# prismformore/Multi-Task-Transformer

Hardware: NVIDIA H100
Metric: images/sec (higher is better)
Workload: dtype bf16x3 (split-bf16 operands, fp32 accumulate)

## Files before the change

multi-task-transformer_b200/csrc/attention5_tc.cu:

```cuda
#include <math.h>

#include "host_common.h"
#include "ptx.cuh"

namespace mtt {

constexpr int kA5ConsumerWGs = 3;
constexpr int kA5Rows = 64 * kA5ConsumerWGs;
constexpr int kA5Threads = 128 + 128 * kA5ConsumerWGs;
constexpr uint32_t kA5QTile = kA5Rows * 64 * 2;
constexpr uint32_t kA5KVTile = 64 * 64 * 2;
constexpr int kA5Stages = 3;

struct Attn5Params {
  int B, N, H, T;
  float scale_log2;
  __nv_bfloat16* out_hi;
  __nv_bfloat16* out_lo;
  float* prompt_logits;
};

template <int NSPLIT>
__global__ void __launch_bounds__(kA5Threads, 1)
attention5_kernel(const __grid_constant__ CUtensorMap tmq_hi, const __grid_constant__ CUtensorMap tmq_lo,
                  const __grid_constant__ CUtensorMap tmk_hi, const __grid_constant__ CUtensorMap tmk_lo,
                  const Attn5Params p) {
  extern __shared__ uint8_t smem_raw[];
  uint8_t* smem = reinterpret_cast<uint8_t*>((reinterpret_cast<uintptr_t>(smem_raw) + 1023) &
                                             ~static_cast<uintptr_t>(1023));
  uint8_t* sQ = smem;
  uint8_t* sK = sQ + NSPLIT * kA5QTile;
  uint8_t* sV = sK + kA5Stages * NSPLIT * kA5KVTile;
  uint64_t* bars = reinterpret_cast<uint64_t*>(sV + kA5Stages * NSPLIT * kA5KVTile);
  uint64_t* q_full = bars;
  uint64_t* k_full = bars + 1;
  uint64_t* k_empty = k_full + kA5Stages;
  uint64_t* v_full = k_empty + kA5Stages;
  uint64_t* v_empty = v_full + kA5Stages;

  const int tid = threadIdx.x;
  const int warp = tid >> 5;
  const int lane = tid & 31;
  const int C = p.H * 64;
  const int nkv = (p.N + 63) / 64;
  const int qt = blockIdx.x / (p.B * p.H);
  const int h = blockIdx.x % p.H;
  const int b = (blockIdx.x / p.H) % p.B;
  const int n_act = min(kA5ConsumerWGs, (p.N - qt * kA5Rows + 63) / 64);

  if (tid == 0) {
    tma_prefetch_desc(&tmq_hi);
    tma_prefetch_desc(&tmk_hi);
    if (NSPLIT == 2) {
      tma_prefetch_desc(&tmq_lo);
      tma_prefetch_desc(&tmk_lo);
    }
    mbar_init(q_full, 1);
    for (int s = 0; s < kA5Stages; ++s) {
      mbar_init(&k_full[s], 1);
      mbar_init(&k_empty[s], 4 * n_act);
      mbar_init(&v_full[s], 1);
      mbar_init(&v_empty[s], 4 * n_act);
    }
    fence_barrier_init();
  }
  __syncthreads();

  if (warp < 4) {
    setmaxnreg_dec<24>();
    if (warp != 0) return;
    if (elect_one()) {
      mbar_arrive_expect_tx(q_full, NSPLIT * kA5QTile);
      tma_load_3d(sQ, &tmq_hi, q_full, h * 64, qt * kA5Rows, b);
      if (NSPLIT == 2) tma_load_3d(sQ + kA5QTile, &tmq_lo, q_full, h * 64, qt * kA5Rows, b);
    }
    __syncwarp();
    for (int j = 0; j < nkv; ++j) {
      const int s = j % kA5Stages;
      const uint32_t ph = (j / kA5Stages) & 1;
      mbar_wait(&k_empty[s], ph ^ 1);
      if (elect_one()) {
        uint8_t* dk = sK + s * NSPLIT * kA5KVTile;
        mbar_arrive_expect_tx(&k_full[s], NSPLIT * kA5KVTile);
        tma_load_3d(dk, &tmk_hi, &k_full[s], C + h * 64, j * 64, b);
        if (NSPLIT == 2) tma_load_3d(dk + kA5KVTile, &tmk_lo, &k_full[s], C + h * 64, j * 64, b);
      }
      __syncwarp();
      mbar_wait(&v_empty[s], ph ^ 1);
      if (elect_one()) {
        uint8_t* dv = sV + s * NSPLIT * kA5KVTile;
        mbar_arrive_expect_tx(&v_full[s], NSPLIT * kA5KVTile);
        tma_load_3d(dv, &tmk_hi, &v_full[s], 2 * C + h * 64, j * 64, b);
        if (NSPLIT == 2) tma_load_3d(dv + kA5KVTile, &tmk_lo, &v_full[s], 2 * C + h * 64, j * 64, b);
      }
      __syncwarp();
    }
    return;
  }

  setmaxnreg_inc<160>();
  const int cw = (warp >> 2) - 1;
  if (cw >= n_act) return;
  const int rloc = cw * 64 + (warp & 3) * 16 + (lane >> 2);
  const int col0 = 2 * (lane & 3);
  const uint32_t q_hi = smem_u32(sQ) + (uint32_t)cw * 64 * 128;
  const uint32_t q_lo = q_hi + kA5QTile;
  const float sl2 = p.scale_log2;

  float o[32];
#pragma unroll
  for (int i = 0; i < 32; ++i) o[i] = 0.f;
  float m_run[2] = {-INFINITY, -INFINITY};
  float l_run[2] = {0.f, 0.f};

  mbar_wait(q_full, 0);
  for (int j = 0; j < nkv; ++j) {
    const int s = j % kA5Stages;
    const uint32_t ph = (j / kA5Stages) & 1;
    const int kn = min(64, p.N - j * 64);

    float sc[32];
#pragma unroll
    for (int i = 0; i < 32; ++i) sc[i] = 0.f;
    mbar_wait(&k_full[s], ph);
    const uint32_t k_hi = smem_u32(sK + s * NSPLIT * kA5KVTile), k_lo = k_hi + kA5KVTile;
    wgmma_fence_regs(sc);
    wgmma_fence();
#pragma unroll
    for (int ks = 0; ks < 4; ++ks) {
      const uint64_t qdh = gmma_desc_sw128(q_hi + ks * 32), kdh = gmma_desc_sw128(k_hi + ks * 32);
      wgmma_ss_n64<0>(sc, qdh, kdh, 1);
      if (NSPLIT == 2) {
        wgmma_ss_n64<0>(sc, qdh, gmma_desc_sw128(k_lo + ks * 32), 1);
        wgmma_ss_n64<0>(sc, gmma_desc_sw128(q_lo + ks * 32), kdh, 1);
      }
    }
    wgmma_commit();
    wgmma_wait<0>();
    wgmma_fence_regs(sc);
    __syncwarp();
    if (lane == 0) mbar_arrive(&k_empty[s]);

    if (p.prompt_logits) {
#pragma unroll
      for (int hh = 0; hh < 2; ++hh) {
        const int q_row = qt * kA5Rows + rloc + 8 * hh;
        if (q_row < p.T) {
          float* ex = p.prompt_logits + (((long long)b * p.H + h) * p.T + q_row) * p.N + j * 64;
#pragma unroll
          for (int i = 0; i < 8; ++i) {
            const int c = 8 * i + col0;
            if (c < kn) ex[c] = sc[4 * i + 2 * hh];
            if (c + 1 < kn) ex[c + 1] = sc[4 * i + 2 * hh + 1];
          }
        }
      }
    }

    float alpha[2];
#pragma unroll
    for (int hh = 0; hh < 2; ++hh) {
      float mx = -INFINITY;
#pragma unroll
      for (int i = 0; i < 8; ++i) {
#pragma unroll
        for (int e = 0; e < 2; ++e) {
          if (8 * i + col0 + e >= kn) sc[4 * i + 2 * hh + e] = -INFINITY;
          mx = fmaxf(mx, sc[4 * i + 2 * hh + e]);
        }
      }
      mx = fmaxf(mx, __shfl_xor_sync(0xffffffffu, mx, 1));
      mx = fmaxf(mx, __shfl_xor_sync(0xffffffffu, mx, 2));
      const float m_new = fmaxf(m_run[hh], mx * sl2);
      alpha[hh] = ex2_approx(m_run[hh] - m_new);
      m_run[hh] = m_new;
      float sum = 0.f;
#pragma unroll
      for (int i = 0; i < 8; ++i) {
#pragma unroll
        for (int e = 0; e < 2; ++e) {
          const float pv = ex2_approx(fmaf(sc[4 * i + 2 * hh + e], sl2, -m_new));
          sc[4 * i + 2 * hh + e] = pv;
          sum += pv;
        }
      }
      l_run[hh] = l_run[hh] * alpha[hh] + sum;
    }

    uint32_t ph_[4][4], pl_[4][4];
#pragma unroll
    for (int kk = 0; kk < 4; ++kk) {
#pragma unroll
      for (int r = 0; r < 4; ++r) {
        const int i = 2 * kk + (r >> 1), hh = r & 1;
        if (NSPLIT == 2) split_pack2(sc[4 * i + 2 * hh], sc[4 * i + 2 * hh + 1], ph_[kk][r], pl_[kk][r]);
        else ph_[kk][r] = pack_bf16x2(sc[4 * i + 2 * hh], sc[4 * i + 2 * hh + 1]);
      }
    }
    mbar_wait(&v_full[s], ph);
    const uint32_t v_hi = smem_u32(sV + s * NSPLIT * kA5KVTile), v_lo = v_hi + kA5KVTile;
    float pvb[32];
#pragma unroll
    for (int i = 0; i < 32; ++i) pvb[i] = 0.f;
    wgmma_fence_regs(pvb);
    wgmma_fence();
#pragma unroll
    for (int kk = 0; kk < 4; ++kk) {
      const uint64_t vdh = gmma_desc_sw128(v_hi + kk * 2048);
      wgmma_rs_n64<1>(pvb, ph_[kk], vdh, kk > 0 ? 1 : 0);
      if (NSPLIT == 2) {
        wgmma_rs_n64<1>(pvb, ph_[kk], gmma_desc_sw128(v_lo + kk * 2048), 1);
        wgmma_rs_n64<1>(pvb, pl_[kk], vdh, 1);
      }
    }
    wgmma_commit();
    wgmma_wait<0>();
    wgmma_fence_regs(pvb);
#pragma unroll
    for (int i = 0; i < 8; ++i)
#pragma unroll
      for (int r = 0; r < 4; ++r) o[4 * i + r] = fmaf(o[4 * i + r], alpha[r >> 1], pvb[4 * i + r]);
    __syncwarp();
    if (lane == 0) mbar_arrive(&v_empty[s]);
  }

#pragma unroll
  for (int hh = 0; hh < 2; ++hh) {
    float l = l_run[hh];
    l += __shfl_xor_sync(0xffffffffu, l, 1);
    l += __shfl_xor_sync(0xffffffffu, l, 2);
    const float inv = 1.0f / l;
    const int q_row = qt * kA5Rows + rloc + 8 * hh;
    if (q_row >= p.N) continue;
    const long long off = ((long long)b * p.N + q_row) * C + h * 64 + col0;
#pragma unroll
    for (int i = 0; i < 8; ++i) {
      uint32_t hv, lv;
      split_pack2(o[4 * i + 2 * hh] * inv, o[4 * i + 2 * hh + 1] * inv, hv, lv);
      *reinterpret_cast<uint32_t*>(p.out_hi + off + 8 * i) = hv;
      if (NSPLIT == 2 || p.out_lo) *reinterpret_cast<uint32_t*>(p.out_lo + off + 8 * i) = lv;
    }
  }
}

template <int NSPLIT>
static int launch_attn5(const CUtensorMap* maps, const Attn5Params& p, cudaStream_t stream) {
  constexpr uint32_t smem = NSPLIT * kA5QTile + 2 * kA5Stages * NSPLIT * kA5KVTile + 1024 + 256;
  static bool attr_set[kMaxDevices] = {};
  const int dev_ = current_device();
  if (!attr_set[dev_]) {
    cudaError_t e = cudaFuncSetAttribute(attention5_kernel<NSPLIT>, cudaFuncAttributeMaxDynamicSharedMemorySize, smem);
    if (e != cudaSuccess)
      return set_error(MTT_ERR_LAUNCH, "attention: cudaFuncSetAttribute: %s", cudaGetErrorString(e));
    attr_set[dev_] = true;
  }
  const int total = ((p.N + kA5Rows - 1) / kA5Rows) * p.H * p.B;
  attention5_kernel<NSPLIT><<<total, kA5Threads, smem, stream>>>(maps[0], maps[1], maps[2], maps[3], p);
  return check_launch("mtt_attention");
}

int launch_attention5(const mtt_attn_desc* d, cudaStream_t stream) {
  const int C = d->H * 64;
  CUtensorMap maps[4];
  const uint64_t dims[3] = {(uint64_t)3 * C, (uint64_t)d->N, (uint64_t)d->B};
  const uint64_t str[2] = {(uint64_t)3 * C * 2, (uint64_t)d->N * 3 * C * 2};
  const uint32_t qbox[3] = {64, kA5Rows, 1};
  const uint32_t kbox[3] = {64, 64, 1};
  int rc;
  if ((rc = make_tmap_bf16(&maps[0], d->qkv_hi, 3, dims, str, qbox))) return rc;
  if ((rc = make_tmap_bf16(&maps[2], d->qkv_hi, 3, dims, str, kbox))) return rc;
  if (d->nsplit == 2) {
    if ((rc = make_tmap_bf16(&maps[1], d->qkv_lo, 3, dims, str, qbox))) return rc;
    if ((rc = make_tmap_bf16(&maps[3], d->qkv_lo, 3, dims, str, kbox))) return rc;
  } else {
    maps[1] = maps[0];
    maps[3] = maps[2];
  }
  Attn5Params p;
  p.B = d->B;
  p.N = d->N;
  p.H = d->H;
  p.T = d->prompt_logits ? d->T : 0;
  p.scale_log2 = d->scale * 1.4426950408889634f;
  p.out_hi = static_cast<__nv_bfloat16*>(d->out_hi);
  p.out_lo = static_cast<__nv_bfloat16*>(d->out_lo);
  p.prompt_logits = d->prompt_logits;
  return d->nsplit == 2 ? launch_attn5<2>(maps, p, stream) : launch_attn5<1>(maps, p, stream);
}

}
```

multi-task-transformer_b200/taskprompter.py:

```python
import math
from types import SimpleNamespace

import torch
import torch.nn as nn

from . import ops
from .plans import (Plan, _cached, _check_input, _dev_ctx, _f32, _lin, _pack_stem, _pack_vit_block, _plan_for,
                    _predict_outputs, _Streams)

PARITY, SPEED = 2, 1


class Mlp(nn.Module):

    def __init__(self, in_features, hidden_features):
        super().__init__()
        self.fc1 = nn.Linear(in_features, hidden_features)
        self.fc2 = nn.Linear(hidden_features, in_features)


class Attention(nn.Module):

    def __init__(self, chan_nheads, resolution, dim, num_heads=8, qkv_bias=False):
        super().__init__()
        self.num_heads = num_heads
        self.dim = dim
        self.resolution = resolution
        self.pixel_no = int(resolution[0] * resolution[1])
        self.chan_nheads = chan_nheads
        self.scale = (dim // num_heads) ** -0.5
        self.qkv = nn.Linear(dim, dim * 3, bias=qkv_bias)
        self.proj = nn.Linear(dim, dim)
        self.token_trans = nn.Linear(dim, self.pixel_no)
        self.token_trans1 = nn.Linear(self.pixel_no, dim)


class _BlockSpace:

    def __init__(self, B, T, gh, gw, C, H, hidden, chan_nheads, device, ns, streams=None):
        self.B, self.T, self.gh, self.gw, self.C, self.H, self.ns, self.dev = B, T, gh, gw, C, H, ns, device
        self.P = P = gh * gw
        self.N = N = T + P
        self.nh = self.nw = int(round(math.sqrt(chan_nheads)))
        S = lambda r, c, **kw: ops.Split(r, c, device, ns, **kw)
        z = lambda *s: torch.zeros(*s, device=device, dtype=torch.float32)
        self.xs = z(B * N, C)
        self.qkv = S(B * N, 3 * C)
        self.ao = S(B * N, C)
        self.logits = z(B, H, T, N)
        self.cp = z(B * T, P)
        self.cps = S(B * T, P)
        self.rc = z(B, T, C, self.nh, self.nw)
        self.ws_qkv = ops.workspace(ops.workspace_bytes(ops._L.OP_LN_QKV, rows=B * N, Cdim=C, nsplit=ns), device)
        self.ws_mlp = ops.workspace(ops.workspace_bytes(ops._L.OP_LN_MLP_RESIDUAL, rows=B * N, Cdim=C, hidden=hidden,
                                                        nsplit=ns), device)
        self.xn = ops.ws_split_view(self.ws_qkv, 0, B * N, C, ns)
        self.streams = streams if streams is not None else _Streams(device, max(T, 1))


def _launch_block(sp, w, want_logits):
    B, N, T = sp.B, sp.N, sp.T
    ops.ln_qkv(sp.xs, w.n1w, w.n1b, w.eps, w.qkv, w.qkv_b, sp.qkv, sp.ws_qkv)
    main, side = sp.streams.fork(1)
    if side[0] is None:
        _launch_chan_path(sp, w, want_logits)
    else:
        with torch.cuda.stream(side[0]):
            _launch_chan_path(sp, w, want_logits)
    ops.attention(sp.qkv, sp.ao, B=B, N=N, H=sp.H, scale=64 ** -0.5,
                  prompt_logits=sp.logits if want_logits else None, T=T)
    sp.streams.join(main, 1)
    ops.proj_residual(sp.ao, w.proj, w.proj_b, sp.xs)
    ops.ln_mlp_residual(sp.xs, w.n2w, w.n2b, w.eps, w.fc1, w.fc1_b, w.fc2, w.fc2_b, sp.ws_mlp)


def prompt_row_chunks(B, T):
    bstep = max(1, 128 // T)
    for b0 in range(0, B, bstep):
        yield b0, min(bstep, B - b0)


def _launch_chan_path(sp, w, want_logits):
    B, N, T, C = sp.B, sp.N, sp.T, sp.C
    for b0, nb in prompt_row_chunks(B, T):
        ops.gemm(sp.xn, w.tt, M=nb * T, bias=w.tt_b, a_gather=(T, N), a_row_offset=b0 * N,
                 out_f32=sp.cp, out_split=sp.cps, regroup=(nb * T, nb * T, b0 * T))
    if want_logits:
        ops.chan_logits(sp.cp, sp.xn, sp.rc, B=B, N=N, T=T, Cdim=C, gh=sp.gh, gw=sp.gw,
                        nh=sp.nh, nw=sp.nw)
    for b0, nb in prompt_row_chunks(B, T):
        ops.gemm(sp.cps, w.tt1, M=nb * T, bias=w.tt1_b, a_row_offset=b0 * T, residual=sp.xs,
                 out_f32=sp.xs, regroup=(T, N, b0 * N))


class Block(nn.Module):

    def __init__(self, chan_nheads, resolution, dim, num_heads, mlp_ratio=4., qkv_bias=False):
        super().__init__()
        self.norm1 = nn.LayerNorm(dim, eps=1e-6)
        self.attn = Attention(chan_nheads, resolution, dim, num_heads=num_heads, qkv_bias=qkv_bias)
        self.norm2 = nn.LayerNorm(dim, eps=1e-6)
        self.mlp = Mlp(dim, int(dim * mlp_ratio))
        self.nsplit = PARITY
        self.emit_logits = True

    def forward(self, x, task_prompts):
        _check_input(self, x)
        B, P, C = x.shape
        T = task_prompts.shape[1]
        a = self.attn
        if P != a.pixel_no or C != a.dim or C // a.num_heads != 64:
            raise ValueError(f"Block: expected x [B,{a.pixel_no},{a.dim}] with head dim 64, got {tuple(x.shape)}")
        dev, ns = x.device, self.nsplit
        with _dev_ctx(dev):
            w = _pack_vit_block(self, dev, ns)
            sp = _cached(self, ("space", dev, ns, B, T), lambda: _BlockSpace(
                B, T, a.resolution[0], a.resolution[1], C, a.num_heads, self.mlp.fc1.out_features, a.chan_nheads, dev,
                ns), versioned=False)
            xs = sp.xs.view(B, sp.N, C)
            xs[:, :T].copy_(task_prompts)
            xs[:, T:].copy_(x)
            _launch_block(sp, w, self.emit_logits)
            attn_weight = (sp.logits.clone(), sp.rc.clone()) if self.emit_logits else (None, None)
            return xs[:, T:].clone(), attn_weight, xs[:, :T].clone()


class PatchEmbed(nn.Module):

    def __init__(self, img_size, patch_size, in_chans, embed_dim):
        super().__init__()
        self.img_size = tuple(img_size)
        self.patch_size = (patch_size, patch_size)
        self.grid_size = (img_size[0] // patch_size, img_size[1] // patch_size)
        self.num_patches = self.grid_size[0] * self.grid_size[1]
        self.proj = nn.Conv2d(in_chans, embed_dim, kernel_size=patch_size, stride=patch_size)


def _trunc_normal_(t, mean=0., std=1., a=-2., b=2.):
    with torch.no_grad():
        return nn.init.trunc_normal_(t, mean=mean, std=std, a=a, b=b)


class TaskPrompter(nn.Module):

    def __init__(self, p, select_list, img_size=(224, 224), patch_size=16, in_chans=3, embed_dim=768, depth=12,
                 num_heads=12, chan_nheads=1, mlp_ratio=4., qkv_bias=True, drop_rate=0., attn_drop_rate=0.,
                 drop_path_rate=0., **_unused):
        super().__init__()
        if isinstance(img_size, int):
            img_size = (img_size, img_size)
        self.p = p
        self.embed_dim = self.num_features = embed_dim
        self.num_heads = num_heads
        self.depth = depth
        self.drop_path_rate = float(drop_path_rate)
        self.patch_size = patch_size
        self.in_chans = in_chans
        self.patch_embed = PatchEmbed(img_size, patch_size, in_chans, embed_dim)
        num_patches = self.patch_embed.num_patches
        self.pos_embed = nn.Parameter(torch.zeros(1, num_patches + 1, embed_dim))
        self.resolution = [img_size[0] // patch_size, img_size[1] // patch_size]
        self.blocks = nn.Sequential(*[
            Block(chan_nheads, self.resolution, embed_dim, num_heads, mlp_ratio, qkv_bias) for _ in range(depth)])
        self.norm = nn.LayerNorm(embed_dim, eps=1e-6)
        self.select_list = list(select_list)
        self.num_layers = 4
        assert len(self.select_list) == self.num_layers - 1
        tasks = list(p.TASKS.NAMES)
        self.pixel_no = num_patches
        self.prompt_len = p.prompt_len
        assert self.prompt_len == 1, "prompt_len != 1 is unsupported (as in the reference's channel branch)"
        self.prompts_len = len(tasks) * p.prompt_len
        self.task_prompts = nn.Parameter(torch.ones(self.prompts_len, embed_dim))
        self.chan_nheads = chan_nheads
        nh = int(round(math.sqrt(chan_nheads)))
        if nh * nh != chan_nheads or self.resolution[0] % nh or self.resolution[1] % nh:
            raise ValueError(f"TaskPrompter: chan_nheads={chan_nheads} must be a perfect square whose root divides the "
                             f"token grid {self.resolution[0]} x {self.resolution[1]}")
        e, f = p.embed_dim, p.final_embed_dim
        prompt_dim = num_heads * p.prompt_len
        self.fea_fuse = nn.ModuleList()
        if p.use_ctr:
            self.ctr_attn_conv = nn.ModuleList()
        self.fea_decode_spa = nn.ModuleList()
        self.fea_decode_chan = nn.ModuleList()
        for _ in range(self.num_layers):
            self.fea_fuse.append(nn.ModuleDict())
            if p.use_ctr:
                self.ctr_attn_conv.append(nn.ModuleDict())
            self.fea_decode_spa.append(nn.ModuleDict())
            self.fea_decode_chan.append(nn.ModuleDict())
            for t in tasks:
                self.fea_fuse[-1][t] = nn.Sequential(nn.Conv2d(e * 2, f, 1), nn.Conv2d(f, f, 3, padding=1),
                                                     nn.BatchNorm2d(f), nn.GELU(), nn.Conv2d(f, f, 1))
                if p.use_ctr:
                    self.ctr_attn_conv[-1][t] = nn.Sequential(nn.Conv2d(prompt_dim, prompt_dim, 1), nn.GELU(),
                                                              nn.Conv2d(prompt_dim, 1, 1))
                self.fea_decode_spa[-1][t] = nn.Sequential(nn.Conv2d(embed_dim, e, 1))
                self.fea_decode_chan[-1][t] = nn.Sequential(nn.Conv2d(embed_dim, e, 1))
        self.nsplit = PARITY
        self.use_graph = False
        self._init_weights()

    def _init_weights(self):
        _trunc_normal_(self.task_prompts, mean=1., std=1.)
        _trunc_normal_(self.pos_embed, std=.02)
        for m in self.modules():
            if isinstance(m, nn.Linear):
                _trunc_normal_(m.weight, std=.02)
                if m.bias is not None:
                    nn.init.zeros_(m.bias)
            elif isinstance(m, (nn.LayerNorm, nn.BatchNorm2d)):
                nn.init.zeros_(m.bias)
                nn.init.ones_(m.weight)

    def forward(self, x):
        _check_input(self, x)
        pl = _plan_for(self, (x.shape[0], x.device, self.nsplit, "backbone"), lambda: _Plan(
            self, None, list(self.p.TASKS.NAMES), None, x.shape[0], x.device, self.nsplit, mode="backbone"))
        out = pl.run(x, graph=self.use_graph)
        return {t: v.clone() for t, v in out.items()}, {}


def _pack_head(hd, device, ns):
    def build():
        f = lambda t: _f32(t, device)
        hw = SimpleNamespace()
        hw.deconv = isinstance(hd.mt_proj[0], nn.ConvTranspose2d)
        if hw.deconv:
            wt = f(hd.mt_proj[0].weight)
            hw.mid = wt.shape[1]
            hw.dc = []
            for dy in range(2):
                for dx in range(2):
                    wp, bp = ops.pack_conv_weight(wt[:, :, dy, dx].contiguous().reshape(wt.shape[0], hw.mid, 1, 1),
                                                  hd.mt_proj[0].bias, hd.mt_proj[1], ns, transposed=True)
                    hw.dc.append((dy, dx, wp, bp))
            hw.mt, hw.mt_b = ops.pack_conv_weight(f(hd.mt_proj[3].weight), hd.mt_proj[3].bias, hd.mt_proj[4], ns)
        else:
            hw.mid = hd.mt_proj[0].weight.shape[0]
            hw.mt, hw.mt_b = ops.pack_conv_weight(f(hd.mt_proj[0].weight), hd.mt_proj[0].bias, hd.mt_proj[1], ns)
        hw.cin = hd.mt_proj[0].weight.shape[0] if hw.deconv else hd.mt_proj[0].weight.shape[1]
        hw.lp, hw.lp_b = _lin(hd.linear_pred, device, ns)
        hw.n_out = hd.linear_pred.weight.shape[0]
        return hw
    return _cached(hd, ("pack", device, ns), build)


class _HeadSpace:

    def __init__(self, hw, B, h, w, device, ns):
        S = lambda r, c, **kw: ops.Split(r, c, device, ns, **kw)
        k = 2 if hw.deconv else 1
        self.B, self.h, self.w, self.ph, self.pw = B, h, w, k * h, k * w
        rows = B * self.ph * self.pw
        self.up = S(B * h * w, hw.cin, zero=True)
        self.hdc = S(rows, hw.mid, zero=True) if hw.deconv else None
        self.hmid = S(rows, hw.mid, zero=True)
        self.pred = torch.zeros(rows, ops.round_up(hw.n_out, 4), device=device, dtype=torch.float32)


def _launch_head(hs, hw):
    B = hs.B
    if hw.deconv:
        for dy, dx, wp, bp in hw.dc:
            ops.gemm(hs.up, wp, N=hw.mid, K=hw.cin, bias=bp, act=ops.ACT_GELU, out_split=hs.hdc,
                     regroup=(hs.w, 4 * hs.w, 2 * hs.w * dy + dx, 2))
        ops.conv3x3_bn_act(hs.hdc, hw.mt, hw.mt_b, hw.mid, hw.mid, ops.ACT_GELU, B=B, H=hs.ph, W=hs.pw, mid=hs.hmid,
                           w_head=hw.lp, b_head=hw.lp_b, n_out=hw.n_out, out_f32=hs.pred)
    else:
        ops.conv3x3_bn_act(hs.up, hw.mt, hw.mt_b, hw.cin, hw.mid, ops.ACT_GELU, B=B, H=hs.ph, W=hs.pw, mid=hs.hmid,
                           w_head=hw.lp, b_head=hw.lp_b, n_out=hw.n_out, out_f32=hs.pred)


class _HeadForward:

    nsplit = PARITY

    def forward(self, x):
        _check_input(self, x)
        B, Cin, h, w = x.shape
        dev, ns = x.device, self.nsplit
        with _dev_ctx(dev):
            hw = _pack_head(self, dev, ns)
            if Cin != hw.cin:
                raise ValueError(f"{type(self).__name__}: expected {hw.cin} input channels, got {Cin}")
            hs = _cached(self, ("space", dev, ns, B, h, w), lambda: _HeadSpace(hw, B, h, w, dev, ns), versioned=False)
            ops.nchw_to_nhwc_split(x.contiguous(), hs.up)
            _launch_head(hs, hw)
            out = torch.empty(B, hw.n_out, hs.ph, hs.pw, device=dev, dtype=torch.float32)
            ops.nhwc_to_nchw(hs.pred, hs.pred.stride(0), B, hw.n_out, hs.ph, hs.pw, out)
            return out


class ConvHead(_HeadForward, nn.Module):

    def __init__(self, in_channels, num_classes):
        super().__init__()
        self.mt_proj = nn.Sequential(nn.Conv2d(in_channels, in_channels, 3, padding=1),
                                     nn.BatchNorm2d(in_channels), nn.GELU())
        _trunc_normal_(self.mt_proj[0].weight, std=0.02)
        self.linear_pred = nn.Conv2d(in_channels, num_classes, kernel_size=1)


class DEConvHead(_HeadForward, nn.Module):

    def __init__(self, in_channels, num_classes):
        super().__init__()
        h2 = in_channels // 2
        self.mt_proj = nn.Sequential(nn.ConvTranspose2d(in_channels, h2, 2, stride=2, padding=0),
                                     nn.BatchNorm2d(h2), nn.GELU(),
                                     nn.Conv2d(h2, h2, 3, padding=1), nn.BatchNorm2d(h2), nn.GELU())
        self.linear_pred = nn.Conv2d(h2, num_classes, kernel_size=1)
        _trunc_normal_(self.mt_proj[0].weight, std=0.02)
        _trunc_normal_(self.mt_proj[3].weight, std=0.02)
        _trunc_normal_(self.linear_pred.weight, std=0.02)


class TaskPrompterWrapper(nn.Module):

    def __init__(self, p, backbone, heads, nsplit=PARITY, use_graph=True):
        super().__init__()
        self.tasks = list(p.TASKS.NAMES)
        self.backbone = backbone
        self.heads = heads
        keys = p.keys() if hasattr(p, "keys") else vars(p).keys()
        self.target_size = tuple(p.dd_label_map_size) if "dd_label_map_size" in keys else None
        self.nsplit = nsplit
        self.use_graph = use_graph
        for t in self.tasks:
            if not isinstance(heads[t], (ConvHead, DEConvHead)):
                raise NotImplementedError(f"mtt_b200: unsupported head {type(heads[t]).__name__} for task {t!r} (the "
                                          "FCOS3D detection head of the reference needs mmdet3d: SURVEY.md 8f N4)")

    def plan(self, batch, device, postproc=False):
        mode = "postproc" if postproc else "full"
        P = _Plan
        if type(self.backbone).__name__ == "TaskPrompterSwin":
            from .taskprompter_swin import _SwinPlan as P
        return _plan_for(self, (int(batch), torch.device(device), int(self.nsplit), mode), lambda: P(
            self.backbone, self.heads, self.tasks, self.target_size, batch, torch.device(device), self.nsplit, mode=mode))

    def forward(self, x):
        _check_input(self, x)
        return self.plan(x.shape[0], x.device).run(x, graph=self.use_graph)

    def predict(self, x):
        _check_input(self, x)
        return self.plan(x.shape[0], x.device, postproc=True).run(x, graph=self.use_graph)


def _pack_fuse(bb, il, t, device, ns):
    f = lambda x: _f32(x, device)
    tw = SimpleNamespace()
    tw.spa, tw.spa_b = _lin(bb.fea_decode_spa[il][t][0], device, ns)
    tw.chan, tw.chan_b = _lin(bb.fea_decode_chan[il][t][0], device, ns)
    fu = bb.fea_fuse[il][t]
    ff, e = fu[0].weight.shape[0], fu[0].weight.shape[1] // 2
    e_pad = ops.round_up(e, 8)
    w0 = f(fu[0].weight).reshape(ff, 2 * e)
    w0p = torch.zeros(ff, 2 * e_pad, device=device)
    w0p[:, :e] = w0[:, :e]
    w0p[:, e_pad:e_pad + e] = w0[:, e:]
    tw.f0, tw.f0_b = ops.pack_weight(w0p, ns), f(fu[0].bias)
    tw.f1, tw.f1_b = ops.pack_conv_weight(f(fu[1].weight), fu[1].bias, fu[2], ns)
    if fu[4].kernel_size == (1, 1):
        tw.f4, tw.f4_b = _lin(fu[4], device, ns)
    else:
        tw.f4, tw.f4_b = ops.pack_conv_weight(f(fu[4].weight), fu[4].bias, None, ns)
    return tw


def _pack_levels(bb, tasks, device, ns):
    def build():
        f = lambda t: _f32(t, device)
        H = bb.num_heads
        levels = []
        for il in range(4):
            lv = SimpleNamespace(tasks=[_pack_fuse(bb, il, t, device, ns) for t in tasks])
            if bb.p.use_ctr:
                cc = [bb.ctr_attn_conv[il][t] for t in tasks]
                lv.c0 = torch.stack([f(c[0].weight).reshape(H, H) for c in cc]).contiguous()
                lv.c0b = torch.stack([f(c[0].bias) for c in cc]).contiguous()
                lv.c2 = torch.stack([f(c[2].weight).reshape(H) for c in cc]).contiguous()
                lv.c2b = torch.stack([f(c[2].bias).reshape(()) for c in cc]).contiguous()
            levels.append(lv)
        return levels
    return _cached(bb, ("levels", device, ns, tuple(tasks)), build)


class _Plan(Plan):

    def __init__(self, bb, heads, tasks, target, B, device, nsplit, mode="full"):
        super().__init__((bb, heads), B, device, nsplit, len(tasks))
        device = self.dev
        self.mode = mode
        self.postproc = mode == "postproc"
        p = bb.p
        self.bb, self.heads = bb, heads
        self.tasks = list(tasks)
        self.T = T = len(self.tasks)
        self.C = C = bb.embed_dim
        self.H = bb.num_heads
        if C // self.H != 64 or C % self.H:
            raise ValueError(f"TaskPrompter: embed_dim / num_heads = {C} / {self.H} must be 64 (mtt_attention is built for "
                             "head dim 64: ViT-B 768 / 12, ViT-L 1024 / 16)")
        self.gh, self.gw = bb.resolution
        self.P = P = self.gh * self.gw
        self.N = N = T + P
        self.patch = bb.patch_size
        self.img = (self.gh * self.patch, self.gw * self.patch)
        self.depth = bb.depth
        self.select = list(bb.select_list)
        self.e, self.f = p.embed_dim, p.final_embed_dim
        self.e_pad = ops.round_up(self.e, 8)
        self.f_ld = ops.round_up(self.f, 8)
        self.use_ctr = bool(p.use_ctr)
        self.target = target
        ns = nsplit
        e_pad, f = self.e_pad, self.f
        with _dev_ctx(device):
            self._repack()
            S = lambda r, c, **kw: ops.Split(r, c, device, ns, **kw)
            z = lambda *s: torch.zeros(*s, device=device, dtype=torch.float32)
            self.cols = S(B * P, self.patch * self.patch * bb.in_chans)
            self.sp = _BlockSpace(B, T, self.gh, self.gw, C, self.H, bb.blocks[0].mlp.fc1.out_features, bb.chan_nheads,
                                  device, ns, streams=self.streams)
            self.nh, self.nw = self.sp.nh, self.sp.nw
            self.xs, self.logits, self.rc = self.sp.xs, self.sp.logits, self.sp.rc
            self.xfin = z(B * N, C)
            self.ws_gate = ops.workspace(ops.workspace_bytes(ops._L.OP_GATED_CONV1X1, rows=B * P, Cdim=C, nsplit=ns, T=T),
                                         device)
            self.cat = [S(B * P, 2 * e_pad, zero=True) for _ in range(T)]
            self.f1 = [S(B * P, f, zero=True) for _ in range(T)]
            self.f2 = [S(B * P, f, zero=True) for _ in range(T)]
            self.acc = z(T, B * P, self.f_ld)
            if self.use_ctr:
                self.F = z(T, B * P, self.f_ld)
                self.ctrw = z(B, T, T)
            gh4, gw4 = 4 * self.gh, 4 * self.gw
            oh, ow = self.target if self.target is not None else self.img
            self.out_hw = (oh, ow)
            if mode == "backbone":
                self.hs = None
                self.out = {t: z(B, f, gh4, gw4) for t in self.tasks}
                return
            self.hs = [_HeadSpace(hw, B, gh4, gw4, device, ns) for hw in self.Wh]
            if self.postproc:
                self.out = _predict_outputs(self.tasks, B, (oh, ow), device)
            else:
                self.out = {t: z(B, hw.n_out, hs.ph, hs.pw) if t == "3ddet" else z(B, hw.n_out, oh, ow)
                            for t, hw, hs in zip(self.tasks, self.Wh, self.hs)}

    def _pack(self):
        bb, dev, ns = self.bb, self.dev, self.ns
        self.Ws = _pack_stem(bb, dev, ns)
        self.Wb = [_pack_vit_block(blk, dev, ns) for blk in bb.blocks]
        self.Wl = _pack_levels(bb, self.tasks, dev, ns)
        self.Wh = [_pack_head(self.heads[t], dev, ns) for t in self.tasks] if self.heads is not None else None

    def _level(self, il, x_src):
        B, N, T, C, P = self.B, self.N, self.T, self.C, self.P
        lv = self.Wl[il]
        first = il == 0
        ops.gated_conv1x1(x_src, N, T, self.logits, self.rc,
                          [(tw.spa, tw.spa_b, tw.chan, tw.chan_b, self.cat[ti]) for ti, tw in enumerate(lv.tasks)],
                          self.e, self.e_pad, self.ws_gate, B=B, T=T, N=N, H=self.H, Cdim=C, gh=self.gh, gw=self.gw,
                          nh=self.nh, nw=self.nw)
        ops.gemm_grouped([(self.cat[ti], tw.f0, dict(bias=tw.f0_b, out_split=self.f1[ti], N=self.f))
                          for ti, tw in enumerate(lv.tasks)])
        ops.gemm_grouped([(self.f1[ti], tw.f1, dict(N=self.f, K=self.f, bias=tw.f1_b, act=ops.ACT_GELU,
                                                    out_split=self.f2[ti], conv=(B, self.gh, self.gw, 3, 1)))
                          for ti, tw in enumerate(lv.tasks)])
        if self.use_ctr:
            ops.gemm_grouped([(self.f2[ti], tw.f4, dict(bias=tw.f4_b, out_f32=self.F[ti][:, :self.f], N=self.f))
                              for ti, tw in enumerate(lv.tasks)])
            ops.ctr_weights(self.logits, lv.c0, lv.c0b, lv.c2, lv.c2b, self.ctrw, B=B, H=self.H, T=T, N=N)
            ops.ctr_mix(self.F, self.ctrw, self.acc, T=T, M=B * P, Cdim=self.f_ld, ld=self.f_ld,
                        rows_per_batch=P, accumulate=not first)
        else:
            ops.gemm_grouped([(self.f2[ti], tw.f4, dict(bias=tw.f4_b, out_f32=self.acc[ti][:, :self.f], N=self.f,
                                                        residual=None if first else self.acc[ti][:, :self.f]))
                              for ti, tw in enumerate(lv.tasks)])

    def _head_chain(self, ti, t, hw, hs):
        B = self.B
        oh, ow = self.out_hw
        ops.bilinear(self.acc[ti], self.f_ld, B, self.gh, self.gw, self.f, hs.h, hs.w, out_split=hs.up)
        _launch_head(hs, hw)
        if t == "3ddet":
            ops.nhwc_to_nchw(hs.pred, hs.pred.stride(0), B, hw.n_out, hs.ph, hs.pw, self.out[t])
        elif self.postproc:
            ops.bilinear_postproc(hs.pred, hs.pred.stride(0), B, hs.ph, hs.pw, hw.n_out, oh, ow,
                                  ops.POSTPROC_KIND[t], self.out[t])
        else:
            ops.bilinear(hs.pred, hs.pred.stride(0), B, hs.ph, hs.pw, hw.n_out, oh, ow, out_nchw=self.out[t])

    def _launch(self, img):
        B, N, T, P = self.B, self.N, self.T, self.P
        W = self.Ws
        ops.im2col_patch(img, self.patch, self.cols)
        ops.gemm(self.cols, W.pe_w, bias=W.pe_b, residual=W.pos, res_row_mod=P, out_f32=self.xs,
                 regroup=(P, N, T))
        ops.broadcast_rows(W.prompts, self.xs, B, N)
        for idx, w in enumerate(self.Wb):
            sel = (idx + 1) in self.select
            _launch_block(self.sp, w, sel or idx == self.depth - 1)
            if sel:
                il = sum(1 for s in self.select if idx >= s - 1) - 1
                self._level(il, self.xs)
        ops.layernorm(self.xs, W.nw, W.nb, W.neps, out_f32=self.xfin)
        self._level(3, self.xfin)
        if self.mode == "backbone":
            gh4, gw4 = 4 * self.gh, 4 * self.gw
            self.streams.par([lambda ti=ti, t=t: ops.bilinear(self.acc[ti], self.f_ld, B, self.gh, self.gw, self.f, gh4,
                                                              gw4, out_nchw=self.out[t])
                              for ti, t in enumerate(self.tasks)])
            return
        self.streams.par([lambda ti=ti, t=t, hw=hw, hs=hs: self._head_chain(ti, t, hw, hs)
                          for ti, (t, hw, hs) in enumerate(zip(self.tasks, self.Wh, self.hs))])


def taskprompter_vit_large_patch16_384(pretrained=False, **kwargs):
    kw = dict(select_list=range(6, 24, 6), patch_size=16, embed_dim=1024, depth=24, num_heads=16,
              chan_nheads=kwargs['p'].chan_nheads)
    kw.update(kwargs)
    return TaskPrompter(**kw)


def taskprompter_vit_base_patch16_384(pretrained=False, **kwargs):
    kw = dict(select_list=range(3, 12, 3), patch_size=16, embed_dim=768, depth=12, num_heads=12,
              chan_nheads=kwargs['p'].chan_nheads)
    kw.update(kwargs)
    return TaskPrompter(**kw)


def build_from_config(cfg, nsplit=PARITY, use_graph=True):
    p = SimpleNamespace(TASKS=SimpleNamespace(NAMES=list(cfg["tasks"]), NUM_OUTPUT=dict(cfg["num_output"])),
                        prompt_len=1, chan_nheads=cfg["chan_nheads"], use_ctr=cfg["use_ctr"],
                        embed_dim=cfg["e"], final_embed_dim=cfg["f"])
    if "dd_label_map_size" in cfg:
        p.dd_label_map_size = tuple(cfg["dd_label_map_size"])
    bb = TaskPrompter(p, cfg["select"], img_size=tuple(cfg["img_size"]), patch_size=cfg["patch"],
                      embed_dim=cfg["C"], depth=cfg["depth"], num_heads=cfg["heads"],
                      chan_nheads=cfg["chan_nheads"], drop_path_rate=cfg.get("drop_path_rate", 0.15))
    head_cls = DEConvHead if cfg.get("head", "conv") == "deconv" else ConvHead
    heads = nn.ModuleDict({t: head_cls(cfg["f"], cfg["num_output"][t]) for t in cfg["tasks"]})
    return TaskPrompterWrapper(p, bb, heads, nsplit=nsplit, use_graph=use_graph)


def accelerate(ref_model, nsplit=PARITY, use_graph=True):
    bb = ref_model.backbone
    p = bb.p
    mine_bb = TaskPrompter(p, list(bb.select_list), img_size=tuple(bb.patch_embed.img_size),
                           patch_size=bb.patch_embed.patch_size[0], embed_dim=bb.embed_dim,
                           depth=len(bb.blocks), num_heads=bb.blocks[0].attn.num_heads,
                           chan_nheads=bb.blocks[0].attn.chan_nheads,
                           drop_path_rate=float(getattr(bb.blocks[-1].drop_path, "drop_prob", 0.0) or 0.0))

    def mirror(t, hd):
        if not hasattr(hd, "mt_proj") or not hasattr(hd, "linear_pred"):
            raise NotImplementedError(f"mtt_b200.accelerate: unsupported head {type(hd).__name__} for task {t!r} "
                                      "(FCOS3DHead / '3ddet' needs mmdet3d: SURVEY.md 8f N4)")
        if isinstance(hd.mt_proj[0], nn.ConvTranspose2d):
            return DEConvHead(hd.mt_proj[0].weight.shape[0], hd.linear_pred.weight.shape[0])
        return ConvHead(hd.linear_pred.weight.shape[1], hd.linear_pred.weight.shape[0])

    heads = nn.ModuleDict({t: mirror(t, ref_model.heads[t]) for t in ref_model.tasks})
    m = TaskPrompterWrapper(p, mine_bb, heads, nsplit=nsplit, use_graph=use_graph)
    m.load_state_dict(ref_model.state_dict(), strict=True)
    return m.eval()
```

Measured before the change: 169.7.

## Overlap chan_logits with proj/MLP and hoist key masking out of softmax loop

```diff
diff --git a/multi-task-transformer_b200/csrc/attention5_tc.cu b/multi-task-transformer_b200/csrc/attention5_tc.cu
--- a/multi-task-transformer_b200/csrc/attention5_tc.cu
+++ b/multi-task-transformer_b200/csrc/attention5_tc.cu
@@ -157,18 +157,21 @@
       }
     }
 
+    if (kn < 64) {
+#pragma unroll
+      for (int i = 0; i < 8; ++i)
+#pragma unroll
+        for (int r = 0; r < 4; ++r)
+          if (8 * i + col0 + (r & 1) >= kn) sc[4 * i + r] = -INFINITY;
+    }
     float alpha[2];
 #pragma unroll
     for (int hh = 0; hh < 2; ++hh) {
       float mx = -INFINITY;
 #pragma unroll
-      for (int i = 0; i < 8; ++i) {
-#pragma unroll
-        for (int e = 0; e < 2; ++e) {
-          if (8 * i + col0 + e >= kn) sc[4 * i + 2 * hh + e] = -INFINITY;
-          mx = fmaxf(mx, sc[4 * i + 2 * hh + e]);
-        }
-      }
+      for (int i = 0; i < 8; ++i)
+#pragma unroll
+        for (int e = 0; e < 2; ++e) mx = fmaxf(mx, sc[4 * i + 2 * hh + e]);
       mx = fmaxf(mx, __shfl_xor_sync(0xffffffffu, mx, 1));
       mx = fmaxf(mx, __shfl_xor_sync(0xffffffffu, mx, 2));
       const float m_new = fmaxf(m_run[hh], mx * sl2);
diff --git a/multi-task-transformer_b200/taskprompter.py b/multi-task-transformer_b200/taskprompter.py
--- a/multi-task-transformer_b200/taskprompter.py
+++ b/multi-task-transformer_b200/taskprompter.py
@@ -63,15 +63,23 @@
     ops.ln_qkv(sp.xs, w.n1w, w.n1b, w.eps, w.qkv, w.qkv_b, sp.qkv, sp.ws_qkv)
     main, side = sp.streams.fork(1)
     if side[0] is None:
-        _launch_chan_path(sp, w, want_logits)
+        _launch_chan_path(sp, w)
+        if want_logits:
+            _launch_chan_logits(sp)
     else:
         with torch.cuda.stream(side[0]):
-            _launch_chan_path(sp, w, want_logits)
+            _launch_chan_path(sp, w)
+            xs_ready = torch.cuda.Event()
+            xs_ready.record(side[0])
+            if want_logits:
+                _launch_chan_logits(sp)
     ops.attention(sp.qkv, sp.ao, B=B, N=N, H=sp.H, scale=64 ** -0.5,
                   prompt_logits=sp.logits if want_logits else None, T=T)
-    sp.streams.join(main, 1)
+    if main is not None:
+        main.wait_event(xs_ready)
     ops.proj_residual(sp.ao, w.proj, w.proj_b, sp.xs)
     ops.ln_mlp_residual(sp.xs, w.n2w, w.n2b, w.eps, w.fc1, w.fc1_b, w.fc2, w.fc2_b, sp.ws_mlp)
+    sp.streams.join(main, 1)
 
 
 def prompt_row_chunks(B, T):
@@ -80,17 +88,19 @@
         yield b0, min(bstep, B - b0)
 
 
-def _launch_chan_path(sp, w, want_logits):
-    B, N, T, C = sp.B, sp.N, sp.T, sp.C
+def _launch_chan_path(sp, w):
+    B, N, T = sp.B, sp.N, sp.T
     for b0, nb in prompt_row_chunks(B, T):
         ops.gemm(sp.xn, w.tt, M=nb * T, bias=w.tt_b, a_gather=(T, N), a_row_offset=b0 * N,
                  out_f32=sp.cp, out_split=sp.cps, regroup=(nb * T, nb * T, b0 * T))
-    if want_logits:
-        ops.chan_logits(sp.cp, sp.xn, sp.rc, B=B, N=N, T=T, Cdim=C, gh=sp.gh, gw=sp.gw,
-                        nh=sp.nh, nw=sp.nw)
     for b0, nb in prompt_row_chunks(B, T):
         ops.gemm(sp.cps, w.tt1, M=nb * T, bias=w.tt1_b, a_row_offset=b0 * T, residual=sp.xs,
                  out_f32=sp.xs, regroup=(T, N, b0 * N))
+
+
+def _launch_chan_logits(sp):
+    ops.chan_logits(sp.cp, sp.xn, sp.rc, B=sp.B, N=sp.N, T=sp.T, Cdim=sp.C, gh=sp.gh, gw=sp.gw,
+                    nh=sp.nh, nw=sp.nw)
 
 
 class Block(nn.Module):
```

New measurement: 170.8 (median of 6 runs). About the same (+0.6%).
